# AllanYangZhou/midGPT

Hardware: AMD Instinct MI355X
Metric: tokens_per_sec (higher is better)
Workload: dtype bf16; 1 GPU; model=openwebtext_xl-gpt-1311M, global_batch=128, seq_len=1024, parallelism=dp1, g_accum_iters=2, remat=False

## Files before the change

midgpt_amd/ops/csrc/attention.hip:

```cpp
#include "common.h"
#include "mfma.h"
#include "philox.h"

struct AttnStrides {
  long b, h;
  int r;
};
DEVINL long bh_base(const AttnStrides& s, long bh, int H) {
  return (bh / H) * s.b + (bh % H) * s.h;
}

template <int C> DEVINL int swz_rm(int row, int byte_in_row) {
  constexpr int M = (C == 128) ? 15 : 7;
  return byte_in_row ^ ((row & M) << 4);
}
DEVINL int swz_tr(int row, int byte_in_row) {
  return byte_in_row ^ (((row >> 2) & 3) << 4);
}

template <int C, int NT>
struct RmStage {
  static constexpr int NV = (32 * C + NT * 8 - 1) / (NT * 8);
  u16x8 v[NV];
  DEVINL void load(const u16* __restrict__ g, int ld = C) {
    static_assert((NT * 8) % C == 0, "a thread keeps its column across loads");
    const int idx0 = threadIdx.x * 8;
    const unsigned boff = 2u * (unsigned)((idx0 / C) * ld + idx0 % C);
#pragma unroll
    for (int i = 0; i < NV; ++i) {
      if (idx0 + i * NT * 8 < 32 * C)
        v[i] = *(const u16x8*)((const char*)(g + (long)(i * (NT * 8 / C)) * ld) + boff);
    }
  }
  DEVINL void write(u16* lds) const {
#pragma unroll
    for (int i = 0; i < NV; ++i) {
      const int idx = threadIdx.x * 8 + i * NT * 8;
      if (idx < 32 * C) {
        const int row = idx / C, col = idx % C;
        *(u16x8*)((char*)lds + row * C * 2 + swz_rm<C>(row, col * 2)) = v[i];
      }
    }
  }
};
template <int C, int NT>
struct TrStage {
  static constexpr int NP = (32 * C + NT * 16 - 1) / (NT * 16);
  u16x8 a[NP], b[NP];
  DEVINL void load(const u16* __restrict__ g, int ld = C) {
    static_assert((NT * 8) % C == 0, "a thread keeps its column across loads");
    const int idx0 = threadIdx.x * 16;
    const unsigned boff =
        2u * (unsigned)(2 * (idx0 / (2 * C)) * ld + (idx0 / 2) % C);
#pragma unroll
    for (int i = 0; i < NP; ++i) {
      if (idx0 + i * NT * 16 >= 32 * C) continue;
      const u16* gi = g + (long)(i * 2 * (NT * 8 / C)) * ld;
      const char* pa = (const char*)gi + boff;
      int ldb = 2 * ld;
      asm volatile("" : "+s"(ldb));
      a[i] = *(const u16x8*)pa;
      b[i] = *(const u16x8*)(pa + ldb);
    }
  }
  DEVINL void write_tr(u16* lds) const {
#pragma unroll
    for (int i = 0; i < NP; ++i) {
      const int idx = threadIdx.x * 16 + i * NT * 16;
      if (idx >= 32 * C) continue;
      const int row = 2 * (idx / (2 * C));
      const int col = (idx / 2) % C;
#pragma unroll
      for (int j = 0; j < 8; ++j) {
        const int r = col + j;
        u16x2 pv; pv.x = a[i][j]; pv.y = b[i][j];
        *(u16x2*)((char*)lds + r * 64 + swz_tr(r, row * 2)) = pv;
      }
    }
  }
  DEVINL void write_rm(u16* lds) const {
#pragma unroll
    for (int i = 0; i < NP; ++i) {
      const int idx = threadIdx.x * 16 + i * NT * 16;
      if (idx >= 32 * C) continue;
      const int row = 2 * (idx / (2 * C));
      const int col = (idx / 2) % C;
      *(u16x8*)((char*)lds + row * C * 2 + swz_rm<C>(row, col * 2)) = a[i];
      *(u16x8*)((char*)lds + (row + 1) * C * 2 + swz_rm<C>(row + 1, col * 2)) = b[i];
    }
  }
};
template <int C, int NT>
DEVINL void stage_rm(const u16* __restrict__ g, u16* lds, int ld = C) {
  RmStage<C, NT> st; st.load(g, ld); st.write(lds);
}
template <int C, int NT>
DEVINL void stage_tr(const u16* __restrict__ g, u16* lds, int ld = C) {
  TrStage<C, NT> st; st.load(g, ld); st.write_tr(lds);
}

template <int C>
DEVINL bf16x8_t read_rm_frag(const u16* lds, int row, int cbyte) {
  return *(const bf16x8_t*)((const char*)lds + row * C * 2 + swz_rm<C>(row, cbyte));
}
DEVINL bf16x8_t read_tr_frag(const u16* lds, int row, int kbyte) {
  return *(const bf16x8_t*)((const char*)lds + row * 64 + swz_tr(row, kbyte));
}

DEVINL float shfl32(float v, int src) { return __shfl(v, src, 32); }

DEVINL bf16x8_t dlayout_to_afrag_keep(const float* s , uint32_t m8) {
  unsigned x[4];
#pragma unroll
  for (int i = 0; i < 4; ++i) {
    const unsigned mk = (((m8 >> (2 * i)) & 1u) ? 0x0000ffffu : 0u) |
                        (((m8 >> (2 * i + 1)) & 1u) ? 0xffff0000u : 0u);
    x[i] = pack_bf16(s[2 * i], s[2 * i + 1]) & mk;
  }
  {
    auto r = __builtin_amdgcn_permlane32_swap(x[0], x[2], false, false);
    x[0] = r[0]; x[2] = r[1];
  }
  {
    auto r = __builtin_amdgcn_permlane32_swap(x[1], x[3], false, false);
    x[1] = r[0]; x[3] = r[1];
  }
  union { unsigned u[4]; bf16x8_t v; } out;
  out.u[0] = x[0]; out.u[1] = x[1]; out.u[2] = x[2]; out.u[3] = x[3];
  return out.v;
}

template <int C, int NW, int SPW, bool DROP = false>
__global__ __launch_bounds__(NW * 64, 2) void attn_fwd_kernel(const u16* __restrict__ q,
                                const u16* __restrict__ k,
                                const u16* __restrict__ v,
                                u16* __restrict__ o, float* __restrict__ lse,
                                int B, int H, int T,
                                AttnStrides sv, AttnStrides so,
                                uint32_t seed_lo = 0, uint32_t seed_hi = 0,
                                uint32_t drop_thr = 0, float inv_keep = 1.f) {
  constexpr int NCB = C / 32;
  constexpr int NCH = C / 16;
  constexpr int NSTRIP = NW * SPW;
  const float scale = rsqrtf((float)C);
  const long bh = blockIdx.x % ((long)B * H);
  const int qb = blockIdx.x / (B * H);
  const int q0 = qb * (NSTRIP * 32);
  const int lane = lane_id();
  const int w = wave_id();
  int strip[SPW];
  strip[0] = w;
  if (SPW == 2) strip[1] = NSTRIP - 1 - w;

// ... 309 lines not shown
    for (int r = 0; r < 16; ++r) {
      const int row = mfma_d_row(lane, r);
      *(float*)((char*)ob + row * 128 + (((lane & 31) * 4) ^ ((row & 7) << 4))) =
          oacc[cb][r] * rrow[r];
    }
    __builtin_amdgcn_s_waitcnt(0);
    const int row = lane & 31;
    const int c16 = 16 * (lane >> 5);
    float tmp[16];
#pragma unroll
    for (int i = 0; i < 4; ++i) {
      f32x4 t = *(const f32x4*)((char*)ob + row * 128 + (((c16 + 4 * i) * 4) ^ ((row & 7) << 4)));
      tmp[4 * i] = t[0]; tmp[4 * i + 1] = t[1]; tmp[4 * i + 2] = t[2]; tmp[4 * i + 3] = t[3];
    }
    u16x8 out0, out1;
#pragma unroll
    for (int j = 0; j < 8; ++j) { out0[j] = f2b(tmp[j]); out1[j] = f2b(tmp[8 + j]); }
    *(u16x8*)(og + (long)row * so.r + 32 * cb + c16) = out0;
    *(u16x8*)(og + (long)row * so.r + 32 * cb + c16 + 8) = out1;
    __builtin_amdgcn_s_waitcnt(0);
  }
}

__global__ void attn_delta_kernel(const u16* __restrict__ dO,
                                  const u16* __restrict__ O,
                                  float* __restrict__ delta, long N, int C,
                                  int H, int T, AttnStrides sdo, AttnStrides so,
                                  u16* __restrict__ do_copy, int bth_order) {
  const int lane = lane_id();
  const long row0 = (long)blockIdx.x * (blockDim.x / WAVE) + wave_id();
  const long rstep = (long)gridDim.x * (blockDim.x / WAVE);
  for (long row = row0; row < N; row += rstep) {
    const unsigned urow = (unsigned)row;
    long bh, t;
    if (bth_order) {
      const unsigned bt = urow / (unsigned)H;
      t = bt % (unsigned)T;
      bh = (long)(bt / (unsigned)T) * H + urow % (unsigned)H;
    } else {
      bh = urow / (unsigned)T;
      t = urow % (unsigned)T;
    }
    const u16* dor = dO + bh_base(sdo, bh, H) + t * sdo.r;
    const u16* orow = O + bh_base(so, bh, H) + t * so.r;
    float acc = 0.f;
    for (int i = lane * 8; i < C; i += WAVE * 8) {
      u16x8 a = *(const u16x8*)(dor + i);
      u16x8 b = *(const u16x8*)(orow + i);
      if (do_copy) *(u16x8*)(do_copy + (bh * T + t) * C + i) = a;
#pragma unroll
      for (int j = 0; j < 8; ++j) acc += b2f(a[j]) * b2f(b[j]);
    }
    acc = group_sum<WAVE>(acc);
    if (lane == 0) delta[bh * T + t] = acc;
  }
}

template <int C, int NW, bool DROP = false>
__global__ __launch_bounds__(NW * 64, 2) void attn_bwd_dkv_kernel(
    const u16* __restrict__ dO, const u16* __restrict__ q,
    const u16* __restrict__ k, const u16* __restrict__ v,
    const float* __restrict__ lse, const float* __restrict__ delta,
    u16* __restrict__ dk, u16* __restrict__ dv, int B, int H, int T,
    AttnStrides sdo, AttnStrides sv, AttnStrides sdv,
    uint32_t seed_lo = 0, uint32_t seed_hi = 0, uint32_t drop_thr = 0,
    float inv_keep = 1.f) {
  constexpr int NCB = C / 32;
  constexpr int NCH = C / 16;
  constexpr int TILE = 4 * 32 * C;
  const float scale = rsqrtf((float)C);
  const long bh = blockIdx.x % ((long)B * H);
  const int kb = blockIdx.x / (B * H);
  const int lane = lane_id();
  const int w = wave_id();
  const int kw0 = kb * (NW * 32) + 32 * w;
  const int myk = kw0 + (lane & 31);

  extern __shared__ __attribute__((aligned(16))) char smem[];
  u16* base = (u16*)smem;
  float* ldsLse = (float*)(base + 2 * TILE);
  float* ldsDelta = ldsLse + 64;

  const u16* qg = q + (bh * T) * C;
  const u16* kg = k + (bh * T) * C;
  const u16* vg = v + bh_base(sv, bh, H);
  const u16* dog = dO + bh_base(sdo, bh, H);
  const u16* krow = kg + (long)myk * C;
  const u16* vrow = vg + (long)myk * sv.r;

  constexpr bool KF_RES = !(DROP && C == 128);
  bf16x8_t kf[KF_RES ? NCH : 1];
  if (KF_RES) {
#pragma unroll
    for (int ch = 0; ch < NCH; ++ch)
      kf[ch] = *(const bf16x8_t*)(krow + 16 * ch + 8 * (lane >> 5));
  }

  f32x16 dvacc[NCB], dkacc[NCB];
#pragma unroll
  for (int cb = 0; cb < NCB; ++cb) { dvacc[cb] = (f32x16)(0.f); dkacc[cb] = (f32x16)(0.f); }

  const int qt0 = kb * NW;
  const int nqt = T / 32;

  auto stage_set = [&](int qt, int buf) {
    const long qbase = (long)qt * 32;
    u16* bq = base + buf * TILE;
    stage_rm<C, NW * 64>(qg + qbase * C, bq);
    stage_tr<C, NW * 64>(qg + qbase * C, bq + 32 * C);
    stage_rm<C, NW * 64>(dog + qbase * sdo.r, bq + 2 * 32 * C, sdo.r);
    stage_tr<C, NW * 64>(dog + qbase * sdo.r, bq + 3 * 32 * C, sdo.r);
    if (threadIdx.x < 32) {
      ldsLse[buf * 32 + threadIdx.x] = lse[bh * T + qbase + threadIdx.x];
      ldsDelta[buf * 32 + threadIdx.x] = delta[bh * T + qbase + threadIdx.x];
    }
  };

  stage_set(qt0, 0);
  __syncthreads();
  TrStage<C, NW * 64> qst, dost;
  float lse_r = 0.f, del_r = 0.f;
  for (int qt = qt0; qt < nqt; ++qt) {
    const int buf = (qt - qt0) & 1;
    const bool pre = qt + 1 < nqt;
    if (pre) {
      const long nb = (long)(qt + 1) * 32;
      qst.load(qg + nb * C);
      dost.load(dog + nb * sdo.r, sdo.r);
      if (threadIdx.x < 32) {
        lse_r = lse[bh * T + nb + threadIdx.x];
        del_r = delta[bh * T + nb + threadIdx.x];
      }
    }
    const int qbase = qt * 32;
    if (qbase + 31 >= kw0) {
      const u16* ldsQ = base + buf * TILE;
      const u16* ldsQt = ldsQ + 32 * C;
      const u16* ldsDO = ldsQt + C * 32;
      const u16* ldsDOt = ldsDO + 32 * C;
      const float* lseb = ldsLse + buf * 32;
      const float* deltab = ldsDelta + buf * 32;
      uint32_t keep = 0;
      if constexpr (DROP) {
#pragma unroll
        for (int g = 0; g < 4; ++g)
          keep |= attn_drop_keep4(seed_lo, seed_hi, (uint32_t)bh,
                                  (uint32_t)(qbase + 8 * g + 4 * (lane >> 5)) >> 2,
                                  (uint32_t)myk, drop_thr) << (4 * g);
        __builtin_amdgcn_sched_barrier(0);
      }
      f32x16 s = (f32x16)(0.f);
#pragma unroll
      for (int ch = 0; ch < NCH; ++ch) {
        bf16x8_t a = read_rm_frag<C>(ldsQ, lane & 31, 16 * ch * 2 + 16 * (lane >> 5));
        bf16x8_t kfr = KF_RES ? kf[ch]
            : *(const bf16x8_t*)(krow + 16 * ch + 8 * (lane >> 5));
        s = mfma_32x32x16_bf16(a, kfr, s);
      }
      float p[16];
#pragma unroll
      for (int r = 0; r < 16; ++r) {
        const int qrow = qbase + mfma_d_row(lane, r);
        p[r] = (myk > qrow) ? 0.f
             : __expf(s[r] * scale - lseb[mfma_d_row(lane, r)]);
      }
      bf16x8_t pf0, pf1;
      if constexpr (DROP) {
        pf0 = dlayout_to_afrag_keep(p, keep);
        pf1 = dlayout_to_afrag_keep(p + 8, keep >> 8);
      } else {
        pf0 = dlayout_to_afrag(p);
        pf1 = dlayout_to_afrag(p + 8);
      }
#pragma unroll
      for (int cb = 0; cb < NCB; ++cb) {
        bf16x8_t b0 = read_tr_frag(ldsDOt, 32 * cb + (lane & 31), 16 * (lane >> 5));
        bf16x8_t b1 = read_tr_frag(ldsDOt, 32 * cb + (lane & 31), 32 + 16 * (lane >> 5));
        dvacc[cb] = mfma_32x32x16_bf16(pf0, b0, dvacc[cb]);
        dvacc[cb] = mfma_32x32x16_bf16(pf1, b1, dvacc[cb]);
      }
      f32x16 dp = (f32x16)(0.f);
#pragma unroll
      for (int ch = 0; ch < NCH; ++ch) {
        bf16x8_t a = read_rm_frag<C>(ldsDO, lane & 31, 16 * ch * 2 + 16 * (lane >> 5));
        bf16x8_t vf = *(const bf16x8_t*)(vrow + 16 * ch + 8 * (lane >> 5));
        dp = mfma_32x32x16_bf16(a, vf, dp);
      }
      float ds[16];
#pragma unroll
      for (int r = 0; r < 16; ++r) {
        float dpr = dp[r];
        if constexpr (DROP) dpr = ((keep >> r) & 1u) ? dpr * inv_keep : 0.f;
        ds[r] = p[r] * (dpr - deltab[mfma_d_row(lane, r)]) * scale;
      }
      bf16x8_t df0 = dlayout_to_afrag(ds);
      bf16x8_t df1 = dlayout_to_afrag(ds + 8);
#pragma unroll
      for (int cb = 0; cb < NCB; ++cb) {
        bf16x8_t b0 = read_tr_frag(ldsQt, 32 * cb + (lane & 31), 16 * (lane >> 5));
        bf16x8_t b1 = read_tr_frag(ldsQt, 32 * cb + (lane & 31), 32 + 16 * (lane >> 5));
        dkacc[cb] = mfma_32x32x16_bf16(df0, b0, dkacc[cb]);
        dkacc[cb] = mfma_32x32x16_bf16(df1, b1, dkacc[cb]);
      }
    }
    if (pre) {
      u16* bq = base + (buf ^ 1) * TILE;
      qst.write_rm(bq);
      qst.write_tr(bq + 32 * C);
      dost.write_rm(bq + 2 * 32 * C);
      dost.write_tr(bq + 3 * 32 * C);
      if (threadIdx.x < 32) {
        ldsLse[(buf ^ 1) * 32 + threadIdx.x] = lse_r;
        ldsDelta[(buf ^ 1) * 32 + threadIdx.x] = del_r;
      }
    }
    __syncthreads();
  }

  float* ob = (float*)smem + w * 32 * 32;
// ... 39 lines not shown
    const u16* __restrict__ dO, const u16* __restrict__ q,
    const u16* __restrict__ k, const u16* __restrict__ v,
    const float* __restrict__ lse, const float* __restrict__ delta,
    u16* __restrict__ dq, int B, int H, int T,
    AttnStrides sdo, AttnStrides sv,
    uint32_t seed_lo = 0, uint32_t seed_hi = 0, uint32_t drop_thr = 0,
    float inv_keep = 1.f) {
  constexpr int NCB = C / 32;
  constexpr int NCH = C / 16;
  constexpr int NSTRIP = NW * SPW;
  constexpr int TILE = 3 * 32 * C;
  const float scale = rsqrtf((float)C);
  const long bh = blockIdx.x % ((long)B * H);
  const int qb = blockIdx.x / (B * H);
  const int q0 = qb * (NSTRIP * 32);
  const int lane = lane_id();
  const int w = wave_id();
  int strip[SPW];
  strip[0] = w;
  if (SPW == 2) strip[1] = NSTRIP - 1 - w;

  extern __shared__ __attribute__((aligned(16))) char smem[];
  u16* base = (u16*)smem;
  u16* ldsDS = base + 2 * TILE;

  const u16* qg = q + (bh * T) * C;
  const u16* kg = k + (bh * T) * C;
  const u16* vg = v + bh_base(sv, bh, H);
  const u16* dog = dO + bh_base(sdo, bh, H);

  constexpr bool QF_RES = !(DROP && C == 128);
  bf16x8_t qf[QF_RES ? NCH : 1];
  f32x16 dqacc[SPW][NCB];
  float mylse[SPW], mydelta[SPW];
#pragma unroll
  for (int sp = 0; sp < SPW; ++sp) {
    const long myq = q0 + 32 * strip[sp] + (lane & 31);
    if (QF_RES && sp == SPW - 1) {
      const u16* qrow = qg + myq * C;
#pragma unroll
      for (int ch = 0; ch < NCH; ++ch)
        qf[ch] = *(const bf16x8_t*)(qrow + 16 * ch + 8 * (lane >> 5));
    }
    mylse[sp] = lse[bh * T + myq];
    mydelta[sp] = delta[bh * T + myq];
#pragma unroll
    for (int cb = 0; cb < NCB; ++cb) dqacc[sp][cb] = (f32x16)(0.f);
  }

  const int nkt = (q0 + NSTRIP * 32) / 32;
  auto stage_set = [&](int kt, int buf) {
    const long k0 = (long)kt * 32;
    u16* bk = base + buf * TILE;
    stage_rm<C, NW * 64>(kg + k0 * C, bk);
    stage_rm<C, NW * 64>(vg + k0 * sv.r, bk + 32 * C, sv.r);
    stage_tr<C, NW * 64>(kg + k0 * C, bk + 2 * 32 * C);
  };
  stage_set(0, 0);
  __syncthreads();
  TrStage<C, NW * 64> kst;
  RmStage<C, NW * 64> vst;
  for (int kt = 0; kt < nkt; ++kt) {
    const int buf = kt & 1;
    const bool pre = kt + 1 < nkt;
    if (pre) {
      kst.load(kg + (long)(kt + 1) * 32 * C);
      vst.load(vg + (long)(kt + 1) * 32 * sv.r, sv.r);
    }
    const int k0 = kt * 32;
    const u16* ldsK = base + buf * TILE;
    const u16* ldsV = ldsK + 32 * C;
    const u16* ldsKt = ldsV + 32 * C;
#pragma unroll
    for (int sp = 0; sp < SPW; ++sp) {
      const int qw0 = q0 + 32 * strip[sp];
      if (k0 > qw0 + 31) continue;
      const u16* qrow = qg + (long)(qw0 + (lane & 31)) * C;
      const u16* dorow = dog + (long)(qw0 + (lane & 31)) * sdo.r;
      uint32_t keep = 0;
      if constexpr (DROP) {
#pragma unroll
        for (int g = 0; g < 4; ++g)
          keep |= attn_drop_keep4(seed_lo, seed_hi, (uint32_t)bh,
                                  (uint32_t)(qw0 + 8 * g + 4 * (lane >> 5)) >> 2,
                                  (uint32_t)(k0 + (lane & 31)), drop_thr) << (4 * g);
        __builtin_amdgcn_sched_barrier(0);
      }
      f32x16 s = (f32x16)(0.f);
      f32x16 dp = (f32x16)(0.f);
#pragma unroll
      for (int ch = 0; ch < NCH; ++ch) {
        bf16x8_t kfrag = read_rm_frag<C>(ldsK, lane & 31, 16 * ch * 2 + 16 * (lane >> 5));
        bf16x8_t qfr = (QF_RES && sp == SPW - 1) ? qf[QF_RES ? ch : 0]
            : *(const bf16x8_t*)(qrow + 16 * ch + 8 * (lane >> 5));
        s = mfma_32x32x16_bf16(qfr, kfrag, s);
        bf16x8_t vfrag = read_rm_frag<C>(ldsV, lane & 31, 16 * ch * 2 + 16 * (lane >> 5));
        bf16x8_t dof = *(const bf16x8_t*)(dorow + 16 * ch + 8 * (lane >> 5));
        dp = mfma_32x32x16_bf16(dof, vfrag, dp);
      }
      float ds[16];
#pragma unroll
      for (int r = 0; r < 16; ++r) {
        const int qrow = qw0 + mfma_d_row(lane, r);
        const float l_r = shfl32(mylse[sp], mfma_d_row(lane, r));
        const float d_r = shfl32(mydelta[sp], mfma_d_row(lane, r));
        const int kcol = k0 + (lane & 31);
        float pv = (kcol > qrow) ? 0.f : __expf(s[r] * scale - l_r);
        float dpr = dp[r];
        if constexpr (DROP) dpr = ((keep >> r) & 1u) ? dpr * inv_keep : 0.f;
        ds[r] = pv * (dpr - d_r) * scale;
      }
      u16* dsl = ldsDS + w * 32 * 32;
#pragma unroll
      for (int r = 0; r < 16; ++r) {
        const int row = mfma_d_row(lane, r);
        *(u16*)((char*)(dsl + row * 32) + swz_tr(row, (lane & 31) * 2)) = f2b(ds[r]);
      }
      __builtin_amdgcn_s_waitcnt(0);
#pragma unroll
      for (int kc = 0; kc < 2; ++kc) {
        bf16x8_t a = *(const bf16x8_t*)((const char*)(dsl + (lane & 31) * 32) +
                                        swz_tr(lane & 31, (16 * kc + 8 * (lane >> 5)) * 2));
#pragma unroll
        for (int cb = 0; cb < NCB; ++cb) {
          bf16x8_t b = read_tr_frag(ldsKt, 32 * cb + (lane & 31),
                                    (16 * kc + 8 * (lane >> 5)) * 2);
          dqacc[sp][cb] = mfma_32x32x16_bf16(a, b, dqacc[sp][cb]);
        }
      }
      __builtin_amdgcn_s_waitcnt(0);
    }
    if (pre) {
      u16* bk = base + (buf ^ 1) * TILE;
      kst.write_rm(bk);
      vst.write(bk + 32 * C);
      kst.write_tr(bk + 2 * 32 * C);
    }
    __syncthreads();
  }

#pragma unroll
  for (int sp = 0; sp < SPW; ++sp) {
    const int qw0 = q0 + 32 * strip[sp];
    float* ob = (float*)smem + w * 32 * 32;
    u16* dqg = dq + (bh * T + qw0) * C;
#pragma unroll
    for (int cb = 0; cb < NCB; ++cb) {
#pragma unroll
      for (int r = 0; r < 16; ++r) {
        const int row = mfma_d_row(lane, r);
        *(float*)((char*)ob + row * 128 + (((lane & 31) * 4) ^ ((row & 7) << 4))) =
            dqacc[sp][cb][r];
      }
// ... 21 lines not shown
```

midgpt_amd/ops/csrc/bindings.cpp:

```cpp
#include <torch/extension.h>
#include <hip/hip_runtime.h>
#include <c10/hip/HIPGuard.h>
#include <c10/hip/HIPStream.h>

#include <algorithm>
#include <climits>
#include <type_traits>
#include <vector>

static hipStream_t cur_stream() { return c10::hip::getCurrentHIPStream().stream(); }

template <typename... P, typename... A>
static void launch(void (*kernel)(P...), dim3 grid, int block, size_t smem, A... args) {
  if (grid.x == 0 || grid.y == 0 || grid.z == 0) return;
  if (smem > 64 * 1024) {
    hipError_t e = hipFuncSetAttribute(reinterpret_cast<const void*>(kernel),
                                       hipFuncAttributeMaxDynamicSharedMemorySize, (int)smem);
    TORCH_CHECK(e == hipSuccess, "cannot raise dynamic LDS to ", smem, " bytes: ",
                hipGetErrorString(e));
  }
  hipLaunchKernelGGL(kernel, grid, dim3(block), smem, cur_stream(), static_cast<P>(args)...);
  hipError_t e = hipGetLastError();
  TORCH_CHECK(e == hipSuccess, "HIP launch failed: ", hipGetErrorString(e));
}
// ... 386 lines not shown
}

static void attn_fwd_launch(const AttnQK& a, const u16* vp, AttnStrides sv, u16* op,
                            AttnStrides so, float* lsep, const MaybeDrop& drop) {
  const int B = a.B, H = a.H, T = a.T;
  const int NW = (T % 256 == 0) ? 8 : 4;
  const long grid = (long)B * H * (T / (NW * 32));
  const DropArgs d = drop.value_or(DropArgs{});
  dispatch_attn(a.C, NW, drop.has_value(), [&](auto c, auto nw, auto dr) {
    constexpr int CC = decltype(c)::value, NN = decltype(nw)::value;
    constexpr bool DROP = decltype(dr)::value;
    constexpr bool PAIRED = CC == 128 && NN == 8 && !DROP;
    const size_t smem = std::max((size_t)((PAIRED ? 8 : 4) * 32 * CC * 2),
                                 (size_t)(NN * 32 * 32 * 4));
    if constexpr (PAIRED)
      launch(attn_fwd2_kernel<CC, NN>, grid, NN * 64, smem, a.q, a.k, vp, op, lsep,
             B, H, T, sv, so);
    else
      launch(attn_fwd_kernel<CC, NN, 1, DROP>, grid, NN * 64, smem, a.q, a.k, vp, op, lsep,
             B, H, T, sv, so, d.seed_lo, d.seed_hi, d.thr, d.inv_keep);
  });
}

static std::vector<torch::Tensor> attn_bwd_launch(
    const AttnQK& a, const u16* dop, AttnStrides sdo, const u16* vp, AttnStrides sv,
    const u16* op, AttnStrides so, const float* lsep, u16* dvp, AttnStrides sdv,
    const MaybeDrop& drop, u16* do_copy = nullptr) {
  const int B = a.B, H = a.H, T = a.T, C = a.C;
  const long N = a.rows();
  TORCH_CHECK(N < (1L << 31), "attn: B*H*T must be below 2^31");
  auto delta = torch::empty({B, H, T}, a.opt.dtype(torch::kFloat));
  const float* deltap = fresh<float>(delta);
  long dgrid = std::min((N + 3) / 4, (long)8192);
  launch(attn_delta_kernel, dgrid, 256, 0, dop, op, fresh<float>(delta), N, C, H, T,
         sdo, so, do_copy, (int)(sdo.h < sdo.r));
  if (do_copy) {
    dop = do_copy;
    sdo = strides_bhtc(H, T, C);
  }
  auto dq = torch::empty({B, H, T, C}, a.opt);
  auto dk = torch::empty({B, H, T, C}, a.opt);
  static const bool nw4 = getenv("MIDGPT_ATTN_DKV_NW4") != nullptr;
  const int NW = (T % 256 == 0 && !(nw4 && !drop)) ? 8 : 4;
  const long grid = (long)B * H * (T / (NW * 32));
  const DropArgs d = drop.value_or(DropArgs{});
  dispatch_attn(C, NW, drop.has_value(), [&](auto c, auto nw, auto dr) {
    constexpr int CC = decltype(c)::value, NN = decltype(nw)::value;
    constexpr bool DROP = decltype(dr)::value;
    const size_t smem_dkv = std::max((size_t)(2 * 4 * 32 * CC) * 2 + 2 * 64 * 4,
                                     (size_t)(NN * 32 * 32 * 4));
    const size_t smem_dq = std::max((size_t)(2 * 3 * 32 * CC) * 2 + NN * 32 * 32 * 2,
                                    (size_t)(NN * 32 * 32 * 4));
    launch(attn_bwd_dkv_kernel<CC, NN, DROP>, grid, NN * 64, smem_dkv, dop, a.q, a.k, vp,
           lsep, deltap, fresh<u16>(dk), dvp, B, H, T, sdo, sv, sdv,
           d.seed_lo, d.seed_hi, d.thr, d.inv_keep);
    launch(attn_bwd_dq_kernel<CC, NN, 1, DROP>, grid, NN * 64, smem_dq, dop, a.q, a.k, vp,
           lsep, deltap, fresh<u16>(dq), B, H, T, sdo, sv,
           d.seed_lo, d.seed_hi, d.thr, d.inv_keep);
  });
  return {dq, dk};
}

static std::vector<torch::Tensor> attn_fwd_bhtc(const char* who, torch::Tensor q,
                                                torch::Tensor k, torch::Tensor v,
                                                const MaybeDrop& drop) {
  Call c(who, q);
  const AttnQK a = attn_qk(c, q, k);
  const u16* vp = c.bf16(v, "v", q.sizes());
  auto o = torch::empty_like(q);
  auto lse = torch::empty({a.B, a.H, a.T}, q.options().dtype(torch::kFloat));
  const AttnStrides st = strides_bhtc(a.H, a.T, a.C);
  attn_fwd_launch(a, vp, st, fresh<u16>(o), st, fresh<float>(lse), drop);
  return {o, lse};
}

// ... 51 lines not shown
  attn_fwd_launch(a, vp, sv, fresh<u16>(o), strides_bthc(a.H, a.T, a.C), fresh<float>(lse),
                  drop_if(p, seed));
  return {o, lse};
}

std::vector<torch::Tensor> attn_bwd_packed(torch::Tensor dO, torch::Tensor q,
                                           torch::Tensor k, torch::Tensor v,
                                           torch::Tensor o, torch::Tensor lse,
                                           torch::Tensor dqkv, double p, int64_t seed,
                                           bool stage_do) {
  Call c("attn_bwd_packed", dO);
  const AttnQK a = attn_qk(c, q, k);
  const int B = a.B, H = a.H, T = a.T, C = a.C;
  AttnStrides sv;
  const u16* vp = packed_or_plain_v(c, a, v, &sv);
  u16* dvp = c.bf16_out(dqkv, "dqkv", {B, T, 3, H, C}) + 2L * H * C;
  const u16 *dop = c.bf16(dO, "dO", {B, T, H, C}), *op = c.bf16(o, "o", {B, T, H, C});
  const float* lsep = c.f32(lse, "lse", flat(a.rows()));
  const AttnStrides sdv = strides_qkv_slot(H, T, C), so = strides_bthc(H, T, C);
  torch::Tensor do_copy;
  if (stage_do) do_copy = torch::empty_like(q);
  return attn_bwd_launch(a, dop, so, vp, sv, op, so, lsep, dvp, sdv, drop_if(p, seed),
                         stage_do ? fresh<u16>(do_copy) : nullptr);
}

torch::Tensor embedding_bwd(torch::Tensor dy, torch::Tensor idx, long V) {
  Call c("embedding_bwd", dy);
  const u16* dyp = c.bf16(dy, "dy", {ANY, ANY});
  long N = dy.size(0);
  int D = c.dim(dy, 1);
  const long* ip = c.i64(idx, "idx", {N});
  TORCH_CHECK(D % 8 == 0, "embedding_bwd: D % 8 == 0");
  if (D % 64 == 0) {
    auto sorted_perm = idx.sort();
    auto sorted = std::get<0>(sorted_perm).contiguous();
    auto perm = std::get<1>(sorted_perm).contiguous();
    auto dw = torch::zeros({V, (long)D}, dy.options());
    const int wpb = 4;
    long grid = (N + wpb - 1) / wpb;
    for (int d0 = 0; d0 < D; d0 += 2048)
      launch(embed_bwd_sorted_kernel, grid, wpb * 64, 0, dyp, fresh<long>(sorted),
             fresh<long>(perm), fresh<u16>(dw), N, D, d0);
    return dw;
  }
  auto dw32 = torch::zeros({V, (long)D}, dy.options().dtype(torch::kFloat));
  long grid = std::min(N, (long)4096);
// ... 477 lines not shown
  Call c("probe_pack", M);
  const float *mp = c.f32(M, "M", {32, 32}), *bp = c.f32(B, "B", {32, 32});
  auto D = torch::zeros({32, 32}, M.options());
  launch(probe_pack_kernel, 1, 64, 0, mp, bp, fresh<float>(D));
  return D;
}

#include "blaslt.inc"

PYBIND11_MODULE(TORCH_EXTENSION_NAME, mod) {
  mod.def("rmsnorm_fwd", &rmsnorm_fwd);
  mod.def("rmsnorm_bwd", &rmsnorm_bwd);
  mod.def("qkv_prep_fwd", &qkv_prep_fwd);
  mod.def("qkv_prep_bwd", &qkv_prep_bwd);
  mod.def("add_rmsnorm_fwd", &add_rmsnorm_fwd);
  mod.def("add_rmsnorm_bwd", &add_rmsnorm_bwd);
  mod.def("qk_prep_fwd", &qk_prep_fwd);
  mod.def("qk_prep_bwd", &qk_prep_bwd);
  mod.def("ce_fwd", &ce_fwd);
  mod.def("ce_bwd", &ce_bwd);
  mod.def("adamw_step", &adamw_step);
  mod.def("attn_fwd", &attn_fwd);
  mod.def("attn_bwd", &attn_bwd);
  mod.def("attn_fwd_dropout", &attn_fwd_dropout);
  mod.def("attn_bwd_dropout", &attn_bwd_dropout);
  mod.def("attn_fwd_packed", &attn_fwd_packed, py::arg("q"), py::arg("k"),
          py::arg("v"), py::arg("p") = 0.0, py::arg("seed") = 0);
  mod.def("attn_bwd_packed", &attn_bwd_packed, py::arg("dO"), py::arg("q"),
          py::arg("k"), py::arg("v"), py::arg("o"), py::arg("lse"),
          py::arg("dqkv"), py::arg("p") = 0.0, py::arg("seed") = 0,
          py::arg("stage_do") = true);
  mod.def("kv_append", &kv_append, py::arg("qkv"), py::arg("qw"), py::arg("kw"),
          py::arg("sin"), py::arg("cos"), py::arg("k_cache"), py::arg("v_cache"),
          py::arg("pos"), py::arg("eps") = 1e-6);
  mod.def("attn_decode", &attn_decode, py::arg("q"), py::arg("k_cache"),
          py::arg("v_cache"), py::arg("kv_len"), py::arg("num_splits") = 0);
  mod.def("kv_append_ragged", &kv_append_ragged, py::arg("qkv"), py::arg("qw"),
          py::arg("kw"), py::arg("sin"), py::arg("cos"), py::arg("k_cache"),
          py::arg("v_cache"), py::arg("pos_dev"), py::arg("pos_host"),
          py::arg("eps") = 1e-6);
  mod.def("attn_decode_ragged", &attn_decode_ragged, py::arg("q"), py::arg("k_cache"),
          py::arg("v_cache"), py::arg("kv_lens_dev"), py::arg("kv_lens_host"),
          py::arg("num_splits") = 0);
  mod.def("kv_append_slots", &kv_append_slots, py::arg("qkv"), py::arg("qw"), py::arg("kw"),
          py::arg("sin"), py::arg("cos"), py::arg("k_cache"), py::arg("v_cache"),
          py::arg("pos_dev"), py::arg("pos_host"), py::arg("slots_dev"),
// ... 32 lines not shown
```

midgpt_amd/ops/csrc/common.h:

```cpp
#pragma once
#include <hip/hip_runtime.h>
#include <cstdint>

#define WAVE 64
#define DEVINL __device__ __forceinline__

using u16 = unsigned short;
using u16x2 = __attribute__((ext_vector_type(2))) unsigned short;
using u16x4 = __attribute__((ext_vector_type(4))) unsigned short;
using u16x8 = __attribute__((ext_vector_type(8))) unsigned short;
using f32x2 = __attribute__((ext_vector_type(2))) float;
using f32x4 = __attribute__((ext_vector_type(4))) float;
using f32x8 = __attribute__((ext_vector_type(8))) float;
using f32x16 = __attribute__((ext_vector_type(16))) float;
using bf16x4 = __attribute__((ext_vector_type(4))) __bf16;
using bf16x8 = __attribute__((ext_vector_type(8))) __bf16;

DEVINL float b2f(u16 h) {
  union { unsigned u; float f; } c;
  c.u = ((unsigned)h) << 16;
  return c.f;
}
DEVINL u16 f2b(float f) {
  union { float f; unsigned u; } c;
  c.f = f;
  unsigned u = c.u;
  unsigned rounded = u + 0x7fffu + ((u >> 16) & 1u);
  if ((u & 0x7fffffffu) > 0x7f800000u) return (u16)((u >> 16) | 0x0040u);
  return (u16)(rounded >> 16);
}

template <int W> DEVINL float group_sum(float x) {
#pragma unroll
// ... 19 lines not shown
```

midgpt_amd/ops/csrc/mfma.h:

```cpp
#pragma once
#include "common.h"

using bf16x8_t = __attribute__((ext_vector_type(8))) __bf16;

DEVINL f32x16 mfma_32x32x16_bf16(bf16x8_t a, bf16x8_t b, f32x16 c) {
  return __builtin_amdgcn_mfma_f32_32x32x16_bf16(a, b, c, 0, 0, 0);
}

DEVINL int mfma_d_row(int lane, int r) {
  return (r & 3) + 8 * (r >> 2) + 4 * (lane >> 5);
}

DEVINL unsigned pack_bf16(float lo, float hi) {
  return ((unsigned)f2b(hi) << 16) | (unsigned)f2b(lo);
}

DEVINL bf16x8_t dlayout_to_afrag(const float* s ) {
  unsigned x0 = pack_bf16(s[0], s[1]);
  unsigned x1 = pack_bf16(s[2], s[3]);
  unsigned x2 = pack_bf16(s[4], s[5]);
  unsigned x3 = pack_bf16(s[6], s[7]);
  {
    auto r = __builtin_amdgcn_permlane32_swap(x0, x2, false, false);
    x0 = r[0]; x2 = r[1];
  }
  {
    auto r = __builtin_amdgcn_permlane32_swap(x1, x3, false, false);
    x1 = r[0]; x3 = r[1];
  }
  union { unsigned u[4]; bf16x8_t v; } out;
  out.u[0] = x0; out.u[1] = x1; out.u[2] = x2; out.u[3] = x3;
  return out.v;
}
```

Before: 109,600 tokens/s.

## Rework attention backward fragment layouts to drop permlane swaps and LDS ds bounce

Permutes the K-dimension order of transposed staging tiles (acc_k_pos) so the MFMA accumulator layout can be packed directly into A/B fragments without permlane32 swaps. The dq kernel swaps MFMA operand order so ds stays in registers instead of round-tripping through LDS. It also caches dO rows, and V and part of K fragments, in LDS rather than reloading them from global memory. The delta kernel now packs several rows per wave. Together these cut shuffles, LDS bounces and redundant global loads, at the cost of more LDS per block, which may reduce occupancy.

```diff
diff --git a/midgpt_amd/ops/csrc/attention.hip b/midgpt_amd/ops/csrc/attention.hip
--- a/midgpt_amd/ops/csrc/attention.hip
+++ b/midgpt_amd/ops/csrc/attention.hip
@@ -43,7 +43,7 @@
     }
   }
 };
-template <int C, int NT>
+template <int C, int NT, bool ACCK = false>
 struct TrStage {
   static constexpr int NP = (32 * C + NT * 16 - 1) / (NT * 16);
   u16x8 a[NP], b[NP];
@@ -59,6 +59,13 @@
       const char* pa = (const char*)gi + boff;
       int ldb = 2 * ld;
       asm volatile("" : "+s"(ldb));
+      if constexpr (ACCK) {
+        unsigned off = boff;
+        asm volatile("" : "+v"(off));
+        a[i] = *(const u16x8*)((const char*)gi + off);
+        b[i] = *(const u16x8*)((const char*)gi + ldb + off);
+        continue;
+      }
       a[i] = *(const u16x8*)pa;
       b[i] = *(const u16x8*)(pa + ldb);
     }
@@ -68,8 +75,24 @@
     for (int i = 0; i < NP; ++i) {
       const int idx = threadIdx.x * 16 + i * NT * 16;
       if (idx >= 32 * C) continue;
-      const int row = 2 * (idx / (2 * C));
+      const int row0 = 2 * (idx / (2 * C));
+      const int row = ACCK ? acc_k_pos(row0) : row0;
       const int col = (idx / 2) % C;
+      if constexpr (ACCK) {
+        const u32x4 aw = __builtin_bit_cast(u32x4, a[i]);
+        const u32x4 bw = __builtin_bit_cast(u32x4, b[i]);
+        const int x = (row * 2) ^ (((col >> 3) & 1) << 5);
+        char* const p0 = (char*)lds + col * 64 + x;
+        char* const p1 = (char*)lds + col * 64 + (x ^ 16);
+#pragma unroll
+        for (int j = 0; j < 8; ++j) {
+          const unsigned pv = (j & 1)
+              ? (aw[j >> 1] >> 16) | (bw[j >> 1] & 0xffff0000u)
+              : (aw[j >> 1] & 0xffffu) | (bw[j >> 1] << 16);
+          *(unsigned*)((j < 4 ? p0 : p1) + j * 64) = pv;
+        }
+        continue;
+      }
 #pragma unroll
       for (int j = 0; j < 8; ++j) {
         const int r = col + j;
@@ -94,9 +117,9 @@
 DEVINL void stage_rm(const u16* __restrict__ g, u16* lds, int ld = C) {
   RmStage<C, NT> st; st.load(g, ld); st.write(lds);
 }
-template <int C, int NT>
+template <int C, int NT, bool ACCK = false>
 DEVINL void stage_tr(const u16* __restrict__ g, u16* lds, int ld = C) {
-  TrStage<C, NT> st; st.load(g, ld); st.write_tr(lds);
+  TrStage<C, NT, ACCK> st; st.load(g, ld); st.write_tr(lds);
 }
 
 template <int C>
@@ -108,27 +131,6 @@
 }
 
 DEVINL float shfl32(float v, int src) { return __shfl(v, src, 32); }
-
-DEVINL bf16x8_t dlayout_to_afrag_keep(const float* s , uint32_t m8) {
-  unsigned x[4];
-#pragma unroll
-  for (int i = 0; i < 4; ++i) {
-    const unsigned mk = (((m8 >> (2 * i)) & 1u) ? 0x0000ffffu : 0u) |
-                        (((m8 >> (2 * i + 1)) & 1u) ? 0xffff0000u : 0u);
-    x[i] = pack_bf16(s[2 * i], s[2 * i + 1]) & mk;
-  }
-  {
-    auto r = __builtin_amdgcn_permlane32_swap(x[0], x[2], false, false);
-    x[0] = r[0]; x[2] = r[1];
-  }
-  {
-    auto r = __builtin_amdgcn_permlane32_swap(x[1], x[3], false, false);
-    x[1] = r[0]; x[3] = r[1];
-  }
-  union { unsigned u[4]; bf16x8_t v; } out;
-  out.u[0] = x[0]; out.u[1] = x[1]; out.u[2] = x[2]; out.u[3] = x[3];
-  return out.v;
-}
 
 template <int C, int NW, int SPW, bool DROP = false>
 __global__ __launch_bounds__(NW * 64, 2) void attn_fwd_kernel(const u16* __restrict__ q,
@@ -484,14 +486,20 @@
   }
 }
 
+template <int C>
 __global__ void attn_delta_kernel(const u16* __restrict__ dO,
                                   const u16* __restrict__ O,
-                                  float* __restrict__ delta, long N, int C,
+                                  float* __restrict__ delta, long N,
                                   int H, int T, AttnStrides sdo, AttnStrides so,
                                   u16* __restrict__ do_copy, int bth_order) {
+  constexpr int LPR = C / 8;
+  constexpr int RPW = WAVE / LPR;
+  static_assert(LPR * 8 == C && RPW * LPR == WAVE, "C/8 must divide the wave");
   const int lane = lane_id();
-  const long row0 = (long)blockIdx.x * (blockDim.x / WAVE) + wave_id();
-  const long rstep = (long)gridDim.x * (blockDim.x / WAVE);
+  const int i = (lane % LPR) * 8;
+  const long row0 =
+      ((long)blockIdx.x * (blockDim.x / WAVE) + wave_id()) * RPW + lane / LPR;
+  const long rstep = (long)gridDim.x * (blockDim.x / WAVE) * RPW;
   for (long row = row0; row < N; row += rstep) {
     const unsigned urow = (unsigned)row;
     long bh, t;
@@ -506,17 +514,20 @@
     const u16* dor = dO + bh_base(sdo, bh, H) + t * sdo.r;
     const u16* orow = O + bh_base(so, bh, H) + t * so.r;
     float acc = 0.f;
-    for (int i = lane * 8; i < C; i += WAVE * 8) {
-      u16x8 a = *(const u16x8*)(dor + i);
-      u16x8 b = *(const u16x8*)(orow + i);
-      if (do_copy) *(u16x8*)(do_copy + (bh * T + t) * C + i) = a;
-#pragma unroll
-      for (int j = 0; j < 8; ++j) acc += b2f(a[j]) * b2f(b[j]);
-    }
-    acc = group_sum<WAVE>(acc);
-    if (lane == 0) delta[bh * T + t] = acc;
-  }
-}
+    const u16x8 a = *(const u16x8*)(dor + i);
+    const u16x8 b = *(const u16x8*)(orow + i);
+    if (do_copy) *(u16x8*)(do_copy + (bh * T + t) * C + i) = a;
+#pragma unroll
+    for (int j = 0; j < 8; ++j) acc += b2f(a[j]) * b2f(b[j]);
+    acc = group_sum<LPR>(acc);
+    if (lane % LPR == 0) delta[bh * T + t] = acc;
+  }
+}
+
+template <int C, int NW>
+constexpr bool attn_dkv_vf_lds = !(C == 128 && NW == 4);
+template <int C, int NW>
+constexpr int attn_dkv_kf_lds = C == 128 ? 3 : 0;
 
 template <int C, int NW, bool DROP = false>
 __global__ __launch_bounds__(NW * 64, 2) void attn_bwd_dkv_kernel(
@@ -542,6 +553,8 @@
   u16* base = (u16*)smem;
   float* ldsLse = (float*)(base + 2 * TILE);
   float* ldsDelta = ldsLse + 64;
+  constexpr bool VF_LDS = attn_dkv_vf_lds<C, NW>;
+  bf16x8_t* ldsVf = (bf16x8_t*)(ldsDelta + 64) + w * (NCH * 64) + lane;
 
   const u16* qg = q + (bh * T) * C;
   const u16* kg = k + (bh * T) * C;
@@ -549,13 +562,25 @@
   const u16* dog = dO + bh_base(sdo, bh, H);
   const u16* krow = kg + (long)myk * C;
   const u16* vrow = vg + (long)myk * sv.r;
+  if constexpr (VF_LDS) {
+#pragma unroll
+    for (int ch = 0; ch < NCH; ++ch)
+      ldsVf[ch * 64] = *(const bf16x8_t*)(vrow + 16 * ch + 8 * (lane >> 5));
+  }
 
   constexpr bool KF_RES = !(DROP && C == 128);
-  bf16x8_t kf[KF_RES ? NCH : 1];
+  constexpr int NKL = KF_RES ? attn_dkv_kf_lds<C, NW> : 0;
+  constexpr int NKR = KF_RES ? NCH - NKL : 0;
+  bf16x8_t kf[NKR ? NKR : 1];
+  bf16x8_t* ldsKf = (bf16x8_t*)(ldsDelta + 64) + (VF_LDS ? NW * (NCH * 64) : 0) +
+                    w * (NKL * 64) + lane;
   if (KF_RES) {
 #pragma unroll
-    for (int ch = 0; ch < NCH; ++ch)
-      kf[ch] = *(const bf16x8_t*)(krow + 16 * ch + 8 * (lane >> 5));
+    for (int ch = 0; ch < NCH; ++ch) {
+      const bf16x8_t f = *(const bf16x8_t*)(krow + 16 * ch + 8 * (lane >> 5));
+      if (ch < NKR) kf[ch < NKR ? ch : 0] = f;
+      else ldsKf[(ch - NKR) * 64] = f;
+    }
   }
 
   f32x16 dvacc[NCB], dkacc[NCB];
@@ -569,9 +594,9 @@
     const long qbase = (long)qt * 32;
     u16* bq = base + buf * TILE;
     stage_rm<C, NW * 64>(qg + qbase * C, bq);
-    stage_tr<C, NW * 64>(qg + qbase * C, bq + 32 * C);
+    stage_tr<C, NW * 64, true>(qg + qbase * C, bq + 32 * C);
     stage_rm<C, NW * 64>(dog + qbase * sdo.r, bq + 2 * 32 * C, sdo.r);
-    stage_tr<C, NW * 64>(dog + qbase * sdo.r, bq + 3 * 32 * C, sdo.r);
+    stage_tr<C, NW * 64, true>(dog + qbase * sdo.r, bq + 3 * 32 * C, sdo.r);
     if (threadIdx.x < 32) {
       ldsLse[buf * 32 + threadIdx.x] = lse[bh * T + qbase + threadIdx.x];
       ldsDelta[buf * 32 + threadIdx.x] = delta[bh * T + qbase + threadIdx.x];
@@ -580,7 +605,8 @@
 
   stage_set(qt0, 0);
   __syncthreads();
-  TrStage<C, NW * 64> qst, dost;
+  __builtin_amdgcn_s_waitcnt(0);
+  TrStage<C, NW * 64, true> qst, dost;
   float lse_r = 0.f, del_r = 0.f;
   for (int qt = qt0; qt < nqt; ++qt) {
     const int buf = (qt - qt0) & 1;
@@ -590,8 +616,10 @@
       qst.load(qg + nb * C);
       dost.load(dog + nb * sdo.r, sdo.r);
       if (threadIdx.x < 32) {
-        lse_r = lse[bh * T + nb + threadIdx.x];
-        del_r = delta[bh * T + nb + threadIdx.x];
+        unsigned off = 4u * threadIdx.x;
+        asm volatile("" : "+v"(off));
+        lse_r = *(const float*)((const char*)(lse + bh * T + nb) + off);
+        del_r = *(const float*)((const char*)(delta + bh * T + nb) + off);
       }
     }
     const int qbase = qt * 32;
@@ -615,25 +643,25 @@
 #pragma unroll
       for (int ch = 0; ch < NCH; ++ch) {
         bf16x8_t a = read_rm_frag<C>(ldsQ, lane & 31, 16 * ch * 2 + 16 * (lane >> 5));
-        bf16x8_t kfr = KF_RES ? kf[ch]
-            : *(const bf16x8_t*)(krow + 16 * ch + 8 * (lane >> 5));
+        bf16x8_t kfr;
+        if constexpr (!KF_RES) kfr = *(const bf16x8_t*)(krow + 16 * ch + 8 * (lane >> 5));
+        else if (ch < NKR) kfr = kf[ch < NKR ? ch : 0];
+        else kfr = ldsKf[(ch - NKR) * 64];
         s = mfma_32x32x16_bf16(a, kfr, s);
       }
       float p[16];
 #pragma unroll
-      for (int r = 0; r < 16; ++r) {
-        const int qrow = qbase + mfma_d_row(lane, r);
-        p[r] = (myk > qrow) ? 0.f
-             : __expf(s[r] * scale - lseb[mfma_d_row(lane, r)]);
-      }
-      bf16x8_t pf0, pf1;
-      if constexpr (DROP) {
-        pf0 = dlayout_to_afrag_keep(p, keep);
-        pf1 = dlayout_to_afrag_keep(p + 8, keep >> 8);
-      } else {
-        pf0 = dlayout_to_afrag(p);
-        pf1 = dlayout_to_afrag(p + 8);
-      }
+      for (int g = 0; g < 4; ++g) {
+        const f32x4 l4 = *(const f32x4*)(lseb + 8 * g + 4 * (lane >> 5));
+#pragma unroll
+        for (int i = 0; i < 4; ++i) {
+          const int r = 4 * g + i;
+          const int qrow = qbase + mfma_d_row(lane, r);
+          p[r] = (myk > qrow) ? 0.f : __expf(s[r] * scale - l4[i]);
+        }
+      }
+      const bf16x8_t pf0 = dlayout_pack(p, DROP ? keep : 0xffu);
+      const bf16x8_t pf1 = dlayout_pack(p + 8, DROP ? keep >> 8 : 0xffu);
 #pragma unroll
       for (int cb = 0; cb < NCB; ++cb) {
         bf16x8_t b0 = read_tr_frag(ldsDOt, 32 * cb + (lane & 31), 16 * (lane >> 5));
@@ -645,18 +673,25 @@
 #pragma unroll
       for (int ch = 0; ch < NCH; ++ch) {
         bf16x8_t a = read_rm_frag<C>(ldsDO, lane & 31, 16 * ch * 2 + 16 * (lane >> 5));
-        bf16x8_t vf = *(const bf16x8_t*)(vrow + 16 * ch + 8 * (lane >> 5));
+        bf16x8_t vf;
+        if constexpr (VF_LDS) vf = ldsVf[ch * 64];
+        else vf = *(const bf16x8_t*)(vrow + 16 * ch + 8 * (lane >> 5));
         dp = mfma_32x32x16_bf16(a, vf, dp);
       }
       float ds[16];
 #pragma unroll
-      for (int r = 0; r < 16; ++r) {
-        float dpr = dp[r];
-        if constexpr (DROP) dpr = ((keep >> r) & 1u) ? dpr * inv_keep : 0.f;
-        ds[r] = p[r] * (dpr - deltab[mfma_d_row(lane, r)]) * scale;
-      }
-      bf16x8_t df0 = dlayout_to_afrag(ds);
-      bf16x8_t df1 = dlayout_to_afrag(ds + 8);
+      for (int g = 0; g < 4; ++g) {
+        const f32x4 d4 = *(const f32x4*)(deltab + 8 * g + 4 * (lane >> 5));
+#pragma unroll
+        for (int i = 0; i < 4; ++i) {
+          const int r = 4 * g + i;
+          float dpr = dp[r];
+          if constexpr (DROP) dpr = ((keep >> r) & 1u) ? dpr * inv_keep : 0.f;
+          ds[r] = p[r] * (dpr - d4[i]) * scale;
+        }
+      }
+      const bf16x8_t df0 = dlayout_pack(ds);
+      const bf16x8_t df1 = dlayout_pack(ds + 8);
 #pragma unroll
       for (int cb = 0; cb < NCB; ++cb) {
         bf16x8_t b0 = read_tr_frag(ldsQt, 32 * cb + (lane & 31), 16 * (lane >> 5));
@@ -742,7 +777,7 @@
 
   extern __shared__ __attribute__((aligned(16))) char smem[];
   u16* base = (u16*)smem;
-  u16* ldsDS = base + 2 * TILE;
+  bf16x8_t* ldsDOf = (bf16x8_t*)(base + 2 * TILE) + w * (SPW * NCH * 64) + lane;
 
   const u16* qg = q + (bh * T) * C;
   const u16* kg = k + (bh * T) * C;
@@ -762,6 +797,10 @@
       for (int ch = 0; ch < NCH; ++ch)
         qf[ch] = *(const bf16x8_t*)(qrow + 16 * ch + 8 * (lane >> 5));
     }
+    const u16* dorow = dog + myq * sdo.r;
+#pragma unroll
+    for (int ch = 0; ch < NCH; ++ch)
+      ldsDOf[(sp * NCH + ch) * 64] = *(const bf16x8_t*)(dorow + 16 * ch + 8 * (lane >> 5));
     mylse[sp] = lse[bh * T + myq];
     mydelta[sp] = delta[bh * T + myq];
 #pragma unroll
@@ -774,11 +813,12 @@
     u16* bk = base + buf * TILE;
     stage_rm<C, NW * 64>(kg + k0 * C, bk);
     stage_rm<C, NW * 64>(vg + k0 * sv.r, bk + 32 * C, sv.r);
-    stage_tr<C, NW * 64>(kg + k0 * C, bk + 2 * 32 * C);
+    stage_tr<C, NW * 64, true>(kg + k0 * C, bk + 2 * 32 * C);
   };
   stage_set(0, 0);
   __syncthreads();
-  TrStage<C, NW * 64> kst;
+  __builtin_amdgcn_s_waitcnt(0);
+  TrStage<C, NW * 64, true> kst;
   RmStage<C, NW * 64> vst;
   for (int kt = 0; kt < nkt; ++kt) {
     const int buf = kt & 1;
@@ -795,15 +835,23 @@
     for (int sp = 0; sp < SPW; ++sp) {
       const int qw0 = q0 + 32 * strip[sp];
       if (k0 > qw0 + 31) continue;
-      const u16* qrow = qg + (long)(qw0 + (lane & 31)) * C;
-      const u16* dorow = dog + (long)(qw0 + (lane & 31)) * sdo.r;
+      const int myq = qw0 + (lane & 31);
+      const u16* qrow = qg + (long)myq * C;
       uint32_t keep = 0;
       if constexpr (DROP) {
-#pragma unroll
-        for (int g = 0; g < 4; ++g)
-          keep |= attn_drop_keep4(seed_lo, seed_hi, (uint32_t)bh,
-                                  (uint32_t)(qw0 + 8 * g + 4 * (lane >> 5)) >> 2,
-                                  (uint32_t)(k0 + (lane & 31)), drop_thr) << (4 * g);
+        const int j = lane & 3;
+        uint32_t mine = 0;
+#pragma unroll
+        for (int c = 0; c < 4; ++c)
+          mine |= attn_drop_keep4(seed_lo, seed_hi, (uint32_t)bh, (uint32_t)myq >> 2,
+                                  (uint32_t)(k0 + c + 8 * j + 4 * (lane >> 5)),
+                                  drop_thr) << (4 * c);
+#pragma unroll
+        for (int g = 0; g < 4; ++g) {
+          const uint32_t mg = (uint32_t)__shfl((int)mine, g, 4);
+#pragma unroll
+          for (int c = 0; c < 4; ++c) keep |= ((mg >> (4 * c + j)) & 1u) << (4 * g + c);
+        }
         __builtin_amdgcn_sched_barrier(0);
       }
       f32x16 s = (f32x16)(0.f);
@@ -813,42 +861,27 @@
         bf16x8_t kfrag = read_rm_frag<C>(ldsK, lane & 31, 16 * ch * 2 + 16 * (lane >> 5));
         bf16x8_t qfr = (QF_RES && sp == SPW - 1) ? qf[QF_RES ? ch : 0]
             : *(const bf16x8_t*)(qrow + 16 * ch + 8 * (lane >> 5));
-        s = mfma_32x32x16_bf16(qfr, kfrag, s);
+        s = mfma_32x32x16_bf16(kfrag, qfr, s);
         bf16x8_t vfrag = read_rm_frag<C>(ldsV, lane & 31, 16 * ch * 2 + 16 * (lane >> 5));
-        bf16x8_t dof = *(const bf16x8_t*)(dorow + 16 * ch + 8 * (lane >> 5));
-        dp = mfma_32x32x16_bf16(dof, vfrag, dp);
+        dp = mfma_32x32x16_bf16(vfrag, ldsDOf[(sp * NCH + ch) * 64], dp);
       }
       float ds[16];
 #pragma unroll
       for (int r = 0; r < 16; ++r) {
-        const int qrow = qw0 + mfma_d_row(lane, r);
-        const float l_r = shfl32(mylse[sp], mfma_d_row(lane, r));
-        const float d_r = shfl32(mydelta[sp], mfma_d_row(lane, r));
-        const int kcol = k0 + (lane & 31);
-        float pv = (kcol > qrow) ? 0.f : __expf(s[r] * scale - l_r);
+        const int krow = k0 + mfma_d_row(lane, r);
+        float pv = (krow > myq) ? 0.f : __expf(s[r] * scale - mylse[sp]);
         float dpr = dp[r];
         if constexpr (DROP) dpr = ((keep >> r) & 1u) ? dpr * inv_keep : 0.f;
-        ds[r] = pv * (dpr - d_r) * scale;
-      }
-      u16* dsl = ldsDS + w * 32 * 32;
-#pragma unroll
-      for (int r = 0; r < 16; ++r) {
-        const int row = mfma_d_row(lane, r);
-        *(u16*)((char*)(dsl + row * 32) + swz_tr(row, (lane & 31) * 2)) = f2b(ds[r]);
-      }
-      __builtin_amdgcn_s_waitcnt(0);
-#pragma unroll
-      for (int kc = 0; kc < 2; ++kc) {
-        bf16x8_t a = *(const bf16x8_t*)((const char*)(dsl + (lane & 31) * 32) +
-                                        swz_tr(lane & 31, (16 * kc + 8 * (lane >> 5)) * 2));
-#pragma unroll
-        for (int cb = 0; cb < NCB; ++cb) {
-          bf16x8_t b = read_tr_frag(ldsKt, 32 * cb + (lane & 31),
-                                    (16 * kc + 8 * (lane >> 5)) * 2);
-          dqacc[sp][cb] = mfma_32x32x16_bf16(a, b, dqacc[sp][cb]);
-        }
-      }
-      __builtin_amdgcn_s_waitcnt(0);
+        ds[r] = pv * (dpr - mydelta[sp]) * scale;
+      }
+      const bf16x8_t a0 = dlayout_pack(ds), a1 = dlayout_pack(ds + 8);
+#pragma unroll
+      for (int cb = 0; cb < NCB; ++cb) {
+        bf16x8_t b0 = read_tr_frag(ldsKt, 32 * cb + (lane & 31), 16 * (lane >> 5));
+        bf16x8_t b1 = read_tr_frag(ldsKt, 32 * cb + (lane & 31), 32 + 16 * (lane >> 5));
+        dqacc[sp][cb] = mfma_32x32x16_bf16(a0, b0, dqacc[sp][cb]);
+        dqacc[sp][cb] = mfma_32x32x16_bf16(a1, b1, dqacc[sp][cb]);
+      }
     }
     if (pre) {
       u16* bk = base + (buf ^ 1) * TILE;
diff --git a/midgpt_amd/ops/csrc/bindings.cpp b/midgpt_amd/ops/csrc/bindings.cpp
--- a/midgpt_amd/ops/csrc/bindings.cpp
+++ b/midgpt_amd/ops/csrc/bindings.cpp
@@ -432,18 +432,27 @@
   });
 }
 
+static void attn_delta_launch(const AttnQK& a, const u16* dop, AttnStrides sdo, const u16* op,
+                              AttnStrides so, float* deltap, u16* do_copy) {
+  const long N = a.rows();
+  TORCH_CHECK(N < (1L << 31), "attn: B*H*T must be below 2^31");
+  dispatch_int<128, 64>(a.C, [&](auto c) {
+    constexpr int CC = decltype(c)::value;
+    constexpr long RPB = 4 * (64 / (CC / 8));
+    const long dgrid = std::min((N + RPB - 1) / RPB, (long)8192);
+    launch(attn_delta_kernel<CC>, dgrid, 256, 0, dop, op, deltap, N, a.H, a.T, sdo, so,
+           do_copy, (int)(sdo.h < sdo.r));
+  });
+}
+
 static std::vector<torch::Tensor> attn_bwd_launch(
     const AttnQK& a, const u16* dop, AttnStrides sdo, const u16* vp, AttnStrides sv,
     const u16* op, AttnStrides so, const float* lsep, u16* dvp, AttnStrides sdv,
     const MaybeDrop& drop, u16* do_copy = nullptr) {
   const int B = a.B, H = a.H, T = a.T, C = a.C;
-  const long N = a.rows();
-  TORCH_CHECK(N < (1L << 31), "attn: B*H*T must be below 2^31");
   auto delta = torch::empty({B, H, T}, a.opt.dtype(torch::kFloat));
   const float* deltap = fresh<float>(delta);
-  long dgrid = std::min((N + 3) / 4, (long)8192);
-  launch(attn_delta_kernel, dgrid, 256, 0, dop, op, fresh<float>(delta), N, C, H, T,
-         sdo, so, do_copy, (int)(sdo.h < sdo.r));
+  attn_delta_launch(a, dop, sdo, op, so, fresh<float>(delta), do_copy);
   if (do_copy) {
     dop = do_copy;
     sdo = strides_bhtc(H, T, C);
@@ -457,10 +466,15 @@
   dispatch_attn(C, NW, drop.has_value(), [&](auto c, auto nw, auto dr) {
     constexpr int CC = decltype(c)::value, NN = decltype(nw)::value;
     constexpr bool DROP = decltype(dr)::value;
-    const size_t smem_dkv = std::max((size_t)(2 * 4 * 32 * CC) * 2 + 2 * 64 * 4,
-                                     (size_t)(NN * 32 * 32 * 4));
-    const size_t smem_dq = std::max((size_t)(2 * 3 * 32 * CC) * 2 + NN * 32 * 32 * 2,
-                                    (size_t)(NN * 32 * 32 * 4));
+    const size_t resident = (size_t)NN * 32 * CC * 2;
+    const size_t smem_dkv = (size_t)(2 * 4 * 32 * CC) * 2 + 2 * 64 * 4 +
+                            (attn_dkv_vf_lds<CC, NN> ? resident : 0) +
+                            (size_t)attn_dkv_kf_lds<CC, NN> * NN * 64 * 16;
+    static_assert((size_t)(2 * 4 * 32 * CC) * 2 >= (size_t)NN * 32 * 32 * 4,
+                  "epilogue bounce fits");
+    const size_t smem_dq = (size_t)(2 * 3 * 32 * CC) * 2 + resident;
+    static_assert((size_t)(2 * 3 * 32 * CC) * 2 + (size_t)NN * 32 * CC * 2 >=
+                  (size_t)NN * 32 * 32 * 4, "epilogue bounce fits");
     launch(attn_bwd_dkv_kernel<CC, NN, DROP>, grid, NN * 64, smem_dkv, dop, a.q, a.k, vp,
            lsep, deltap, fresh<u16>(dk), dvp, B, H, T, sdo, sv, sdv,
            d.seed_lo, d.seed_hi, d.thr, d.inv_keep);
@@ -558,6 +572,25 @@
   if (stage_do) do_copy = torch::empty_like(q);
   return attn_bwd_launch(a, dop, so, vp, sv, op, so, lsep, dvp, sdv, drop_if(p, seed),
                          stage_do ? fresh<u16>(do_copy) : nullptr);
+}
+
+std::vector<torch::Tensor> attn_delta(torch::Tensor dO, torch::Tensor o, bool bthc) {
+  Call c("attn_delta", dO);
+  const u16* dop = c.bf16(dO, "dO", {ANY, ANY, ANY, ANY});
+  const u16* op = c.bf16(o, "o", dO.sizes());
+  const int d1 = c.dim(dO, 1), d2 = c.dim(dO, 2), C = c.dim(dO, 3);
+  const int H = bthc ? d2 : d1, T = bthc ? d1 : d2;
+  TORCH_CHECK(C == 64 || C == 128, "attn_delta: head dim 64 or 128 (got ", C, ")");
+  const AttnQK a{c.dim(dO, 0), H, T, C, nullptr, nullptr, dO.options()};
+  const AttnStrides st = bthc ? strides_bthc(H, T, C) : strides_bhtc(H, T, C);
+  auto delta = torch::empty({a.B, H, T}, dO.options().dtype(torch::kFloat));
+  if (!bthc) {
+    attn_delta_launch(a, dop, st, op, st, fresh<float>(delta), nullptr);
+    return {delta};
+  }
+  auto do_copy = torch::empty({a.B, H, T, C}, dO.options());
+  attn_delta_launch(a, dop, st, op, st, fresh<float>(delta), fresh<u16>(do_copy));
+  return {delta, do_copy};
 }
 
 torch::Tensor embedding_bwd(torch::Tensor dy, torch::Tensor idx, long V) {
@@ -1081,6 +1114,7 @@
   mod.def("adamw_step", &adamw_step);
   mod.def("attn_fwd", &attn_fwd);
   mod.def("attn_bwd", &attn_bwd);
+  mod.def("attn_delta", &attn_delta, py::arg("dO"), py::arg("o"), py::arg("bthc"));
   mod.def("attn_fwd_dropout", &attn_fwd_dropout);
   mod.def("attn_bwd_dropout", &attn_bwd_dropout);
   mod.def("attn_fwd_packed", &attn_fwd_packed, py::arg("q"), py::arg("k"),
diff --git a/midgpt_amd/ops/csrc/common.h b/midgpt_amd/ops/csrc/common.h
--- a/midgpt_amd/ops/csrc/common.h
+++ b/midgpt_amd/ops/csrc/common.h
@@ -9,6 +9,7 @@
 using u16x2 = __attribute__((ext_vector_type(2))) unsigned short;
 using u16x4 = __attribute__((ext_vector_type(4))) unsigned short;
 using u16x8 = __attribute__((ext_vector_type(8))) unsigned short;
+using u32x4 = __attribute__((ext_vector_type(4))) unsigned;
 using f32x2 = __attribute__((ext_vector_type(2))) float;
 using f32x4 = __attribute__((ext_vector_type(4))) float;
 using f32x8 = __attribute__((ext_vector_type(8))) float;
diff --git a/midgpt_amd/ops/csrc/mfma.h b/midgpt_amd/ops/csrc/mfma.h
--- a/midgpt_amd/ops/csrc/mfma.h
+++ b/midgpt_amd/ops/csrc/mfma.h
@@ -13,6 +13,21 @@
 
 DEVINL unsigned pack_bf16(float lo, float hi) {
   return ((unsigned)f2b(hi) << 16) | (unsigned)f2b(lo);
+}
+
+DEVINL int acc_k_pos(int i) {
+  return (i & ~12) | ((i & 4) << 1) | ((i & 8) >> 1);
+}
+
+DEVINL bf16x8_t dlayout_pack(const float* s , unsigned keep8 = 0xffu) {
+  union { unsigned u[4]; bf16x8_t v; } out;
+#pragma unroll
+  for (int i = 0; i < 4; ++i) {
+    const unsigned mk = (((keep8 >> (2 * i)) & 1u) ? 0x0000ffffu : 0u) |
+                        (((keep8 >> (2 * i + 1)) & 1u) ? 0xffff0000u : 0u);
+    out.u[i] = pack_bf16(s[2 * i], s[2 * i + 1]) & mk;
+  }
+  return out.v;
 }
 
 DEVINL bf16x8_t dlayout_to_afrag(const float* s ) {
```

After: 121,200 tokens/s, median of 6. 1.11x the previous value.
